# nvidia-cosmos/cosmos-curate

Hardware: AMD Instinct MI355X
Metric: clips/sec + embedded frames/sec, 1080p30 H.264, 1/2/4/8 MI355X (higher is better)
Workload: dtype bf16; 1 GPU; split_pipeline 1xMI355X: HIP NV12->RGB/resize + CLIP-ViT-B/32 MFMA bf16 (decode seam excluded: no librocdecode in image); model=vit_b32, frames_per_clip=21, src=1080p30 NV12 in HBM, resolution=224, parallelism=dp1

## Files before the change

### cosmos_curate_amd/csrc/cc_attn.hip

```cpp

#include <hip/hip_runtime.h>

#include <vector>

#include "cc_common.hpp"
#include "cc_timing.hpp"

namespace {

typedef __attribute__((ext_vector_type(8))) __bf16 bf16x8;
typedef __attribute__((ext_vector_type(4))) float f32x4;

constexpr int SMAX = 64;
constexpr int HD = 64;
constexpr int LD = 72;

__global__ __launch_bounds__(256, 2) void k_attn_small(
    const __bf16* __restrict__ qkv, __bf16* __restrict__ out, long n_frames,
    int seq, int heads, int hidden, float scale) {
  const long fh = blockIdx.x;
  const long frame = fh / heads;
  const int head = fh % heads;
  if (frame >= n_frames) return;

// ... 370 lines not shown
        m_run[reg] = mx;
#pragma unroll
        for (int nn = 0; nn < 4; nn++) acc[nn][reg] = sv[nn];
      }
    }
    {
      const int colr = lane & 15;
      const int rb = 16 * wid + rbase_l;
#pragma unroll
      for (int nn = 0; nn < 4; nn++)
#pragma unroll
        for (int reg = 0; reg < 4; reg++)
          P[(rb + reg) * LDF + nn * 16 + colr] = (__bf16)acc[nn][reg];
    }
    __syncthreads();

    f32x4 pv[4] = {};
    {
      const int prow = 16 * wid + (lane & 15);
      const int j0 = 8 * (lane >> 4);
#pragma unroll
      for (int kk = 0; kk < FKV; kk += 32) {
        bf16x8 pf = *(const bf16x8*)(P + prow * LDF + kk + j0);
#pragma unroll
        for (int n = 0; n < 4; n++) {
          bf16x8 vf =
              *(const bf16x8*)(Vt + (n * 16 + (lane & 15)) * LDF + kk + j0);
          pv[n] = __builtin_amdgcn_mfma_f32_16x16x32_bf16(pf, vf, pv[n], 0, 0, 0);
        }
      }
    }
#pragma unroll
    for (int n = 0; n < 4; n++)
#pragma unroll
      for (int reg = 0; reg < 4; reg++)
        oacc[n][reg] = oacc[n][reg] * alpha[reg] + pv[n][reg];
  }

  {
    const int dcol = lane & 15;
    const int rb = 16 * wid + rbase_l;
#pragma unroll
    for (int nn = 0; nn < 4; nn++)
#pragma unroll
      for (int reg = 0; reg < 4; reg++) {
        const int row = q0 + rb + reg;
        if (row < seq)
          out[(frame * seq + row) * (long)hidden + head * HD + nn * 16 + dcol] =
              (__bf16)(oacc[nn][reg] / l_run[reg]);
      }
  }
}

}

extern "C" int cc_attn_small(const void* qkv, void* out, int64_t n_frames,
                             int seq, int heads, int hidden, float scale,
                             uint64_t stream) {
  if (!qkv || !out || n_frames <= 0 || seq <= 0)
    return cc::set_error(CC_ERR_INVALID, "bad attn args");
  if (seq > SMAX || hidden != heads * HD)
    return cc::set_error(CC_ERR_UNSUPPORTED,
                         "cc_attn_small needs seq <= 64 and hd == 64");
  dim3 block(256), grid((unsigned)(n_frames * heads));
  hipEvent_t ev0, ev1;
  bool timed = cc::timed_begin(stream, &ev0, &ev1);
  hipLaunchKernelGGL(k_attn_small, grid, block, 0, (hipStream_t)stream,
                     (const __bf16*)qkv, (__bf16*)out, (long)n_frames, seq,
                     heads, hidden, scale);
  hipError_t e = hipGetLastError();
  if (timed) cc::timed_end("attn_small", stream, ev0, ev1);
  if (e != hipSuccess)
    return cc::set_error(CC_ERR_HIP, "attn launch: %s", hipGetErrorString(e));
  return CC_OK;
}

extern "C" int cc_attn_mid(const void* qkv, void* out, int64_t n_frames,
                           int seq, int heads, int hidden, float scale,
                           uint64_t stream) {
  if (!qkv || !out || n_frames <= 0 || seq <= 0)
    return cc::set_error(CC_ERR_INVALID, "bad attn args");
  if (seq <= SMAX || seq > SMID || hidden != heads * HD)
    return cc::set_error(CC_ERR_UNSUPPORTED,
                         "cc_attn_mid needs 64 < seq <= 288 and hd == 64");
  dim3 block(256), grid((unsigned)(n_frames * heads));
  hipEvent_t ev0, ev1;
  bool timed = cc::timed_begin(stream, &ev0, &ev1);
  hipLaunchKernelGGL(k_attn_mid, grid, block, 0, (hipStream_t)stream,
                     (const __bf16*)qkv, (__bf16*)out, (long)n_frames, seq,
                     heads, hidden, scale);
  hipError_t e = hipGetLastError();
  if (timed) cc::timed_end("attn_mid", stream, ev0, ev1);
  if (e != hipSuccess)
    return cc::set_error(CC_ERR_HIP, "attn_mid launch: %s", hipGetErrorString(e));
  return CC_OK;
}

extern "C" int cc_attn_flash(const void* qkv, void* out, int64_t n_frames,
                             int seq, int heads, int hidden, float scale,
                             uint64_t stream) {
  if (!qkv || !out || n_frames <= 0 || seq <= 0)
    return cc::set_error(CC_ERR_INVALID, "bad attn args");
  if (seq <= SMID || hidden != heads * HD)
    return cc::set_error(CC_ERR_UNSUPPORTED,
                         "cc_attn_flash is for seq > 288 with hd == 64 "
                         "(use attn_small/attn_mid below that)");
// ... 14 lines not shown
```

### cosmos_curate_amd/csrc/cc_gemm.hip

```cpp

#include <hip/hip_runtime.h>

#include <cstdlib>
#include <vector>

#include "cc_common.hpp"
#include "cc_timing.hpp"

#define CC_CHECK_HIP(expr)                                                   \
  do {                                                                       \
    hipError_t _e = (expr);                                                  \
    if (_e != hipSuccess)                                                    \
      return cc::set_error(CC_ERR_HIP, "%s failed: %s", #expr,               \
                           hipGetErrorString(_e));                           \
  } while (0)

namespace {

typedef __attribute__((ext_vector_type(8))) __bf16 bf16x8;
typedef __attribute__((ext_vector_type(4))) float f32x4;
typedef __attribute__((ext_vector_type(16))) float f32x16;

constexpr int BM = 128, BN = 128, BK = 64;
constexpr int WM = 64, WN = 64;
// ... 1 lines not shown
constexpr int MFR = WM / FRAG;
constexpr int NFR = WN / FRAG;

__device__ __forceinline__ unsigned short f32_to_bf16_rne(float v) {
  union {
    float f;
    unsigned int u;
  } cv{v};
  unsigned int lsb = (cv.u >> 16) & 1;
  return (unsigned short)((cv.u + 0x7fffu + lsb) >> 16);
}

template <int ACT>
__device__ __forceinline__ float cc_act(float v) {
  if constexpr (ACT == 1)
    return v * __builtin_amdgcn_rcpf(1.0f + __expf(-1.702f * v));
  if constexpr (ACT == 2) {
    float z = 0.7978845608028654f * (v + 0.044715f * v * v * v);
    float t = 1.0f - 2.0f * __builtin_amdgcn_rcpf(__expf(2.0f * z) + 1.0f);
    return 0.5f * v * (1.0f + t);
  }
  return v;
}

__device__ __forceinline__ void stage_slice(const __bf16* __restrict__ src,
                                            long ld, long row0, long row_limit,
                                            long k0, __bf16* lds_base,
                                            int lane) {
  const int lrow8 = lane >> 3;
  const int slot = lane & 7;
  const int gk16 = slot ^ lrow8;
#pragma unroll
  for (int j = 0; j < 4; j++) {
    long grow = row0 + j * 8 + lrow8;
    grow = grow < 0 ? 0 : (grow >= row_limit ? row_limit - 1 : grow);
    const __bf16* gptr = src + grow * ld + k0 + (long)gk16 * 8;
    __builtin_amdgcn_global_load_lds(
        (const __attribute__((address_space(1))) unsigned int*)gptr,
        (__attribute__((address_space(3))) unsigned int*)(lds_base + j * 8 * BK),
        16, 0, 0);
  }
}

__device__ __forceinline__ bf16x8 frag_read(const __bf16* tile, int row,
                                            int k16) {
  int slot = k16 ^ (row & 7);
  return *(const bf16x8*)(tile + (long)row * BK + slot * 8);
}

template <int ACT, bool HAS_BIAS, bool HAS_RES>
__global__ __launch_bounds__(256, 2) void k_gemm_bf16(
    const __bf16* __restrict__ A, const __bf16* __restrict__ B,
    void* __restrict__ C, const float* __restrict__ bias,
    const __bf16* __restrict__ residual, long M, long N, long K,
    int c_is_bf16, int nbx, int nwg, int do_remap) {
  __shared__ __bf16 lds[2 * (BM + BN) * BK];
#define AS(b) (lds + (b) * (BM * BK))
#define BS(b) (lds + 2 * (BM * BK) + (b) * (BN * BK))

  const int tid = threadIdx.x;
  const int lane = tid & 63;
  const int wid = tid >> 6;
  const int waveM = wid >> 1, waveN = wid & 1;

  int orig = blockIdx.x;
  if (do_remap) {
    int q = nwg >> 3, r = nwg & 7;
    int xcd = orig & 7, lid = orig >> 3;
    orig = (xcd < r ? xcd * (q + 1) : r * (q + 1) + (xcd - r) * q) + lid;
  }
  const long bm = (long)(orig / nbx) * BM;
  const long bn = (long)(orig % nbx) * BN;

  const long arow0 = bm + 32 * wid;
  const long brow0 = bn + 32 * wid;

  f32x4 acc[MFR][NFR] = {};

  const long KT = K / BK;
  stage_slice(A, K, arow0, M, 0, AS(0) + 32 * wid * BK, lane);
  stage_slice(B, K, brow0, N, 0, BS(0) + 32 * wid * BK, lane);

  const int arow_frag = waveM * WM + (lane & 15);
  const int brow_frag = waveN * WN + (lane & 15);
  int buf = 0;
  for (long kt = 0; kt < KT; ++kt) {
    asm volatile("s_waitcnt vmcnt(0)" ::: "memory");
    __syncthreads();
    const __bf16* At = AS(buf);
    const __bf16* Bt = BS(buf);
    bf16x8 afrag[2][MFR], bfrag[2][NFR];
#pragma unroll
    for (int g = 0; g < 2; g++) {
      const int k16 = (g << 2) + (lane >> 4);
#pragma unroll
      for (int m = 0; m < MFR; m++)
        afrag[g][m] = frag_read(At, arow_frag + m * FRAG, k16);
#pragma unroll
      for (int n = 0; n < NFR; n++)
        bfrag[g][n] = frag_read(Bt, brow_frag + n * FRAG, k16);
    }
    if (kt + 1 < KT) {
      const long k0 = (kt + 1) * BK;
      stage_slice(A, K, arow0, M, k0, AS(buf ^ 1) + 32 * wid * BK, lane);
      stage_slice(B, K, brow0, N, k0, BS(buf ^ 1) + 32 * wid * BK, lane);
    }
#pragma unroll
    for (int g = 0; g < 2; g++)
#pragma unroll
      for (int m = 0; m < MFR; m++)
#pragma unroll
        for (int n = 0; n < NFR; n++)
          acc[m][n] = __builtin_amdgcn_mfma_f32_16x16x32_bf16(
              afrag[g][m], bfrag[g][n], acc[m][n], 0, 0, 0);
    buf ^= 1;
  }

  const long crow_base = bm + waveM * WM + 4 * (lane >> 4);
  const long ccol_base = bn + waveN * WN + (lane & 15);
  const bool interior = (bm + BM <= M) && (bn + BN <= N);
  if (interior) {
#pragma unroll
    for (int m = 0; m < MFR; m++) {
#pragma unroll
      for (int n = 0; n < NFR; n++) {
        const long col = ccol_base + n * FRAG;
        float bval = 0.0f;
        if constexpr (HAS_BIAS) bval = bias[col];
        float rv[4];
        if constexpr (HAS_RES) {
#pragma unroll
          for (int r = 0; r < 4; r++)
            rv[r] = (float)residual[(crow_base + m * FRAG + r) * N + col];
        }
#pragma unroll
        for (int r = 0; r < 4; r++) {
          const long row = crow_base + m * FRAG + r;
          float v = acc[m][n][r] + bval;
          if (ACT == 1) v = v * __builtin_amdgcn_rcpf(1.0f + __expf(-1.702f * v));
          if (ACT == 2) {
            float z = 0.7978845608028654f * (v + 0.044715f * v * v * v);
            float t = 1.0f - 2.0f * __builtin_amdgcn_rcpf(__expf(2.0f * z) + 1.0f);
            v = 0.5f * v * (1.0f + t);
          }
          if constexpr (HAS_RES) v += rv[r];
          if (c_is_bf16)
            ((unsigned short*)C)[row * N + col] = f32_to_bf16_rne(v);
          else
            ((float*)C)[row * N + col] = v;
        }
      }
    }
    return;
  }
#pragma unroll
  for (int m = 0; m < MFR; m++) {
#pragma unroll
    for (int n = 0; n < NFR; n++) {
      const long col = ccol_base + n * FRAG;
      if (col >= N) continue;
      float bval = 0.0f;
      if constexpr (HAS_BIAS) bval = bias[col];
#pragma unroll
      for (int r = 0; r < 4; r++) {
        const long row = crow_base + m * FRAG + r;
        if (row >= M) continue;
        float v = acc[m][n][r] + bval;
        if (ACT == 1) v = v * __builtin_amdgcn_rcpf(1.0f + __expf(-1.702f * v));
        if (ACT == 2) {
          float z = 0.7978845608028654f * (v + 0.044715f * v * v * v);
          float t = 1.0f - 2.0f * __builtin_amdgcn_rcpf(__expf(2.0f * z) + 1.0f);
          v = 0.5f * v * (1.0f + t);
        }
        if constexpr (HAS_RES) v += (float)residual[row * N + col];
        if (c_is_bf16)
          ((unsigned short*)C)[row * N + col] = f32_to_bf16_rne(v);
        else
          ((float*)C)[row * N + col] = v;
      }
    }
  }
}

template <int ACT, bool HAS_BIAS, bool HAS_RES>
__global__ __launch_bounds__(256, 2) void k_gemm_bf16_w32(
    const __bf16* __restrict__ A, const __bf16* __restrict__ B,
    void* __restrict__ C, const float* __restrict__ bias,
    const __bf16* __restrict__ residual, long M, long N, long K,
    int c_is_bf16, int nbx, int nwg, int do_remap) {
  __shared__ __bf16 lds[2 * (BM + BN) * BK];
#define AS32(b) (lds + (b) * (BM * BK))
#define BS32(b) (lds + 2 * (BM * BK) + (b) * (BN * BK))
  const int tid = threadIdx.x;
  const int lane = tid & 63;
  const int wid = tid >> 6;
  const int waveM = wid >> 1, waveN = wid & 1;

  int orig = blockIdx.x;
  if (do_remap) {
    int q = nwg >> 3, r = nwg & 7;
    int xcd = orig & 7, lid = orig >> 3;
    orig = (xcd < r ? xcd * (q + 1) : r * (q + 1) + (xcd - r) * q) + lid;
  }
  const long bm = (long)(orig / nbx) * BM;
  const long bn = (long)(orig % nbx) * BN;
  const long arow0 = bm + 32 * wid;
  const long brow0 = bn + 32 * wid;

  f32x16 acc[2][2] = {};
  const long KT = K / BK;
  stage_slice(A, K, arow0, M, 0, AS32(0) + 32 * wid * BK, lane);
  stage_slice(B, K, brow0, N, 0, BS32(0) + 32 * wid * BK, lane);
  const int arow = waveM * WM + (lane & 31);
  const int brow = waveN * WN + (lane & 31);
  int buf = 0;
  for (long kt = 0; kt < KT; ++kt) {
    asm volatile("s_waitcnt vmcnt(0)" ::: "memory");
    __syncthreads();
    if (kt + 1 < KT) {
      const long k0 = (kt + 1) * BK;
      stage_slice(A, K, arow0, M, k0, AS32(buf ^ 1) + 32 * wid * BK, lane);
      stage_slice(B, K, brow0, N, k0, BS32(buf ^ 1) + 32 * wid * BK, lane);
    }
    const __bf16* At = AS32(buf);
    const __bf16* Bt = BS32(buf);
#pragma unroll
    for (int kk = 0; kk < BK; kk += 16) {
// ... 315 lines not shown
          bf16x8 v8 = *(const bf16x8*)(slice + elem);
          if constexpr (HAS_RES) {
            const bf16x8 r8 =
                *(const bf16x8*)(residual + grow * N + gcol);
#pragma unroll
            for (int e = 0; e < 8; e++)
              v8[e] = (__bf16)((float)v8[e] + (float)r8[e]);
          }
          *(bf16x8*)((__bf16*)C + grow * N + gcol) = v8;
        }
      }
    } else {
      const bool interior = (ebm + BM2 <= M) && (ebn + BN2 <= N);
      float bhoist2[NFR2] = {};
      if constexpr (HAS_BIAS) {
#pragma unroll
        for (int n = 0; n < NFR2; n++) {
          const long col = ccol_base + n * FRAG;
          bhoist2[n] = (interior || col < N) ? bias[col] : 0.0f;
        }
      }
#pragma unroll
      for (int m = 0; m < MFR2; m++) {
#pragma unroll
        for (int n = 0; n < NFR2; n++) {
          const long col = ccol_base + n * FRAG;
          if (!interior && col >= N) continue;
          const float bval = bhoist2[n];
#pragma unroll
          for (int r = 0; r < 4; r++) {
            const long row = crow_base + m * FRAG + r;
            if (!interior && row >= M) continue;
            float v = cc_act<ACT>(acc[m][n][r] + bval);
            if constexpr (HAS_RES) v += (float)residual[row * N + col];
            if (c_is_bf16)
              ((unsigned short*)C)[row * N + col] = f32_to_bf16_rne(v);
            else
              ((float*)C)[row * N + col] = v;
          }
        }
      }
    }
  }
#undef A2T
#undef B2T
#undef STAGE_A2
#undef STAGE_B2
#undef PHASE_MFMA2
#undef READ_A2
#undef READ_B2
#undef KTILE2
}

}

extern "C" int cc_gemm_bf16_ex(const void* A, const void* B, void* C,
                               int64_t M, int64_t N, int64_t K,
                               const float* bias, int c_dtype, int act,
                               const void* residual, uint64_t stream) {
  if (!A || !B || !C || M <= 0 || N <= 0 || K <= 0)
    return cc::set_error(CC_ERR_INVALID, "bad gemm args");
  if (K % BK != 0)
    return cc::set_error(CC_ERR_UNSUPPORTED,
                         "cc_gemm_bf16 requires K %% 64 == 0 (got %lld)",
                         (long long)K);
  int nbx = (int)((N + BN - 1) / BN);
  int nby = (int)((M + BM - 1) / BM);
  int nwg = nbx * nby;
  dim3 block(256);
  dim3 grid(nwg);
  hipEvent_t ev0 = nullptr, ev1 = nullptr;
  bool timed = cc::timed_begin(stream, &ev0, &ev1);
  static const int wide_env = [] {
    const char* e = getenv("CC_GEMM_WIDE");
    return e ? atoi(e) : -1;
  }();
  const bool wide = wide_env >= 0 ? wide_env != 0 : false;
  static const int tile_env = [] {
    const char* e = getenv("CC_GEMM_TILE");
    return e ? atoi(e) : -1;
  }();
  const bool t256_ok = (K % 128 == 0) && (K >= 256) && M > BM2 / 2;
  const int nbx2 = (int)((N + BN2 - 1) / BN2);
  const int nby2 = (int)((M + BM2 - 1) / BM2);
  const int nwg2 = nbx2 * nby2;
  const bool t256 =
      !wide && t256_ok &&
      (tile_env >= 0 ? tile_env != 0
                     : (K >= 1536 || N >= 1536 || nwg2 >= 256));
  const bool hb = bias != nullptr;
  const bool hr = residual != nullptr;
  int remap = ((M * N) > (48LL << 20)) ? 1 : 0;
  if (t256) {
    nbx = nbx2;
    nby = nby2;
    nwg = nwg2;
    static const int persist_env = [] {
      const char* e = getenv("CC_GEMM_PERSIST");
      return e ? atoi(e) : 1;
    }();
    grid = dim3(persist_env && nwg > 256 ? 256 : nwg);
    block = dim3(512);
    remap = nbx <= 16 ? 1 : 0;
  }
  static const int epi_env = [] {
    const char* e = getenv("CC_GEMM_EPI");
    return e ? atoi(e) : -1;
  }();
  const int epi_auto = (bias != nullptr || residual != nullptr || act != 0) ? 1 : 0;
  const bool epi_staged = (epi_env >= 0 ? epi_env : epi_auto) != 0;
#define CC_LAUNCH_GEMM(KER, A_, HB, HR)                                       \
  hipLaunchKernelGGL((KER<A_, HB, HR>), grid, block, 0, (hipStream_t)stream,  \
                     (const __bf16*)A, (const __bf16*)B, C, bias,             \
                     (const __bf16*)residual, (long)M, (long)N, (long)K,      \
                     c_dtype == 1 ? 1 : 0, nbx, nwg, remap)
#define CC_LAUNCH_T256(A_, HB, HR)                                            \
  do {                                                                        \
    if (epi_staged)                                                           \
      hipLaunchKernelGGL((k_gemm_bf16_t256<A_, HB, HR, true>), grid, block,   \
                         0, (hipStream_t)stream, (const __bf16*)A,            \
                         (const __bf16*)B, C, bias, (const __bf16*)residual,  \
                         (long)M, (long)N, (long)K, c_dtype == 1 ? 1 : 0,     \
                         nbx, nwg, remap);                                    \
    else                                                                      \
      hipLaunchKernelGGL((k_gemm_bf16_t256<A_, HB, HR, false>), grid, block,  \
                         0, (hipStream_t)stream, (const __bf16*)A,            \
                         (const __bf16*)B, C, bias, (const __bf16*)residual,  \
                         (long)M, (long)N, (long)K, c_dtype == 1 ? 1 : 0,     \
                         nbx, nwg, remap);                                    \
  } while (0)
#define CC_DISPATCH_ACT(KER, A_)                                              \
  do {                                                                        \
    if (hb && hr) CC_LAUNCH_GEMM(KER, A_, true, true);                        \
    else if (hb) CC_LAUNCH_GEMM(KER, A_, true, false);                        \
    else if (hr) CC_LAUNCH_GEMM(KER, A_, false, true);                        \
    else CC_LAUNCH_GEMM(KER, A_, false, false);                               \
  } while (0)
#define CC_DISPATCH(KER)                                                      \
  do {                                                                        \
    if (act == 1) CC_DISPATCH_ACT(KER, 1);                                    \
    else if (act == 2) CC_DISPATCH_ACT(KER, 2);       \
    else CC_DISPATCH_ACT(KER, 0);                                             \
  } while (0)
  if (wide)
    CC_DISPATCH(k_gemm_bf16_w32);
  else if (t256) {
#define CC_DISPATCH_ACT_T256(A_)                                              \
  do {                                                                        \
    if (hb && hr) CC_LAUNCH_T256(A_, true, true);                             \
    else if (hb) CC_LAUNCH_T256(A_, true, false);                             \
    else if (hr) CC_LAUNCH_T256(A_, false, true);                             \
    else CC_LAUNCH_T256(A_, false, false);                                    \
  } while (0)
    if (act == 1) CC_DISPATCH_ACT_T256(1);
    else if (act == 2) CC_DISPATCH_ACT_T256(2);
    else CC_DISPATCH_ACT_T256(0);
#undef CC_DISPATCH_ACT_T256
  } else
    CC_DISPATCH(k_gemm_bf16);
#undef CC_DISPATCH
#undef CC_DISPATCH_ACT
#undef CC_LAUNCH_GEMM
  hipError_t e = hipGetLastError();
  if (timed) cc::timed_end("gemm_bf16", stream, ev0, ev1);
  if (e != hipSuccess)
    return cc::set_error(CC_ERR_HIP, "gemm launch: %s", hipGetErrorString(e));
  return CC_OK;
}

extern "C" int cc_gemm_bf16(const void* A, const void* B, void* C, int64_t M,
                            int64_t N, int64_t K, const float* bias,
                            int c_dtype, uint64_t stream) {
  return cc_gemm_bf16_ex(A, B, C, M, N, K, bias, c_dtype, 0, nullptr, stream);
}
```

### cosmos_curate_amd/hotpath.py

```python

from __future__ import annotations

import ctypes
import pathlib

import numpy as np
import numpy.typing as npt

_LIB_PATH = pathlib.Path(__file__).resolve().parent / "lib" / "libcchot.so"
_lib: ctypes.CDLL | None = None


class HotpathUnavailableError(RuntimeError):
    """libcchot.so missing or unusable — the product GPU path must not run."""


def _declare(lib: ctypes.CDLL) -> None:
    c = ctypes
    lib.cc_last_error.restype = c.c_char_p
    lib.cc_hip_available.restype = c.c_int
    lib.cc_rocdecode_available.restype = c.c_int

    lib.cc_demux_open.argtypes = [c.c_char_p, c.c_size_t, c.POINTER(c.c_void_p)]
    lib.cc_demux_probe.argtypes = [c.c_void_p, c.c_void_p]
    lib.cc_demux_timestamps.argtypes = [
        c.c_void_p, c.c_void_p, c.c_size_t, c.POINTER(c.c_size_t)]
    lib.cc_demux_packet.argtypes = [
        c.c_void_p, c.c_size_t, c.POINTER(c.c_void_p), c.POINTER(c.c_size_t),
        c.POINTER(c.c_int64), c.POINTER(c.c_int32)]
    lib.cc_demux_close.argtypes = [c.c_void_p]
    lib.cc_demux_remux_clip.argtypes = [
        c.c_void_p, c.c_double, c.c_double, c.POINTER(c.c_void_p),
        c.POINTER(c.c_size_t)]
    lib.cc_buffer_free.argtypes = [c.c_void_p]

    lib.cc_decode_session_create.argtypes = [
        c.c_int, c.c_int32, c.POINTER(c.c_void_p)]
    lib.cc_decode_submit.argtypes = [
        c.c_void_p, c.c_char_p, c.c_size_t, c.c_int64]
    lib.cc_decode_map_frames.argtypes = [
        c.c_void_p, c.c_void_p, c.c_size_t, c.POINTER(c.c_size_t)]
    lib.cc_decode_recycle.argtypes = [c.c_void_p]
    lib.cc_decode_destroy.argtypes = [c.c_void_p]

    lib.cc_malloc.argtypes = [c.POINTER(c.c_void_p), c.c_size_t]
    lib.cc_free.argtypes = [c.c_void_p]
    lib.cc_memcpy_h2d.argtypes = [c.c_void_p, c.c_void_p, c.c_size_t, c.c_uint64]
    lib.cc_memcpy_d2h.argtypes = [c.c_void_p, c.c_void_p, c.c_size_t, c.c_uint64]
    lib.cc_stream_sync.argtypes = [c.c_uint64]

    lib.cc_nv12_to_rgb.argtypes = [
        c.c_void_p, c.c_void_p, c.c_int, c.c_int, c.c_int, c.c_size_t,
        c.c_void_p, c.c_uint64]
    lib.cc_nv12_to_rgb_resize.argtypes = [
        c.c_void_p, c.c_void_p, c.c_int, c.c_int, c.c_int, c.c_size_t,
        c.c_void_p, c.c_int, c.c_int, c.c_uint64]
    lib.cc_resize_bilinear_u8.argtypes = [
        c.c_void_p, c.c_int, c.c_int, c.c_int, c.c_void_p, c.c_int, c.c_int,
        c.c_uint64]
    lib.cc_resize_bicubic_u8.argtypes = lib.cc_resize_bilinear_u8.argtypes
    lib.cc_clip_preprocess.argtypes = [
        c.c_void_p, c.c_int, c.c_int, c.c_int, c.POINTER(c.c_float),
        c.POINTER(c.c_float), c.c_void_p, c.c_int, c.c_uint64]
    lib.cc_clip_preprocess_patches.argtypes = [
        c.c_void_p, c.c_int, c.c_int, c.c_int, c.c_int, c.c_int,
        c.POINTER(c.c_float), c.POINTER(c.c_float), c.c_void_p, c.c_uint64]
    lib.cc_gather_frames_u8.argtypes = [
        c.c_void_p, c.c_int, c.c_size_t, c.c_void_p, c.c_void_p, c.c_int,
        c.c_int, c.c_void_p, c.c_uint64]
    lib.cc_gemm_bf16.argtypes = [
        c.c_void_p, c.c_void_p, c.c_void_p, c.c_int64, c.c_int64, c.c_int64,
        c.c_void_p, c.c_int, c.c_uint64]
    lib.cc_gemm_bf16_ex.argtypes = [
        c.c_void_p, c.c_void_p, c.c_void_p, c.c_int64, c.c_int64, c.c_int64,
        c.c_void_p, c.c_int, c.c_int, c.c_void_p, c.c_uint64]

    lib.cc_attn_small.argtypes = [
        c.c_void_p, c.c_void_p, c.c_int64, c.c_int, c.c_int, c.c_int,
        c.c_float, c.c_uint64]
    lib.cc_attn_mid.argtypes = lib.cc_attn_small.argtypes
    lib.cc_attn_flash.argtypes = lib.cc_attn_small.argtypes
    lib.cc_layernorm_bf16.argtypes = [
        c.c_void_p, c.c_void_p, c.c_void_p, c.c_void_p, c.c_int64, c.c_int64,
        c.c_float, c.c_uint64]
    lib.cc_embed_assemble_ln.argtypes = [
        c.c_void_p, c.c_void_p, c.c_void_p, c.c_void_p, c.c_void_p,
        c.c_void_p, c.c_int64, c.c_int64, c.c_int64, c.c_float, c.c_uint64]
    lib.cc_pairwise_max_earlier.argtypes = [
        c.c_void_p, c.c_int64, c.c_int64, c.c_void_p, c.c_void_p, c.c_uint64]

    lib.cc_timing_enable.argtypes = [c.c_int]
    lib.cc_timing_report.argtypes = [
        c.c_char_p, c.POINTER(c.c_double), c.POINTER(c.c_int64)]


def load() -> ctypes.CDLL:
    global _lib
    if _lib is None:
        if not _LIB_PATH.exists():
            raise HotpathUnavailableError(
                f"{_LIB_PATH} not built — run python -m cosmos_curate_amd.build"
            )
        _lib = ctypes.CDLL(str(_LIB_PATH))
        _declare(_lib)
    return _lib


def available() -> bool:
    try:
        load()
    except HotpathUnavailableError:
        return False
    return True


def require_gpu() -> ctypes.CDLL:
    lib = load()
    rc = lib.cc_hip_available()
    if rc != 0:
        raise HotpathUnavailableError(
            f"HIP device unavailable: {lib.cc_last_error().decode()}"
        )
    return lib


def check(rc: int) -> None:
    if rc != 0:
        lib = load()
        raise RuntimeError(f"cc error {rc}: {lib.cc_last_error().decode()}")
# ... 147 lines not shown
```

### cosmos_curate_amd/models/clip_vit.py

```python

from __future__ import annotations

import ctypes
import math

import torch

from cosmos_curate_amd import hotpath
from cosmos_curate_amd.models import clip_weights as cw


def _cc_linear(
    x: torch.Tensor,
    w_bf16: torch.Tensor,
    bias_f32: torch.Tensor | None,
    act: int = 0,
    residual: torch.Tensor | None = None,
) -> torch.Tensor:
    lib = hotpath.require_gpu()
    assert x.dtype == torch.bfloat16 and w_bf16.dtype == torch.bfloat16
    x = x.contiguous()
    M, K = x.shape
    N = w_bf16.shape[0]
    out = torch.empty((M, N), dtype=torch.bfloat16, device=x.device)
    stream = torch.cuda.current_stream(x.device).cuda_stream
    if residual is not None:
        residual = residual.contiguous()
        assert residual.shape == out.shape and residual.dtype == torch.bfloat16
    hotpath.check(
        lib.cc_gemm_bf16_ex(
            x.data_ptr(), w_bf16.data_ptr(), out.data_ptr(), M, N, K,
            bias_f32.data_ptr() if bias_f32 is not None else None,
            1, act, residual.data_ptr() if residual is not None else None,
            stream,
        )
    )
    return out


class ClipVisionTowerAMD(torch.nn.Module):

    def __init__(
        self,
        state_dict: dict[str, torch.Tensor] | None = None,
        cfg: cw.VitConfig = cw.VIT_B32,
    ) -> None:
        super().__init__()
        self.cfg = cfg
        if state_dict is None:
            state_dict = (
                cw.make_clip_vit_b32_weights() if cfg is cw.VIT_B32
                else cw.make_clip_vit_weights(cfg)
            )
        sd = state_dict
        p = "vision_model."
        reg = self.register_buffer
        to_bf = lambda t: t.to(torch.bfloat16).contiguous()

        k0 = 3 * cfg.patch * cfg.patch
        self.patch_k = (k0 + 63) // 64 * 64
        reg("cls_emb", sd[p + "embeddings.class_embedding"].clone())
        w_patch = sd[p + "embeddings.patch_embedding.weight"].reshape(cfg.hidden, k0)
        if self.patch_k != k0:
            w_patch = torch.nn.functional.pad(w_patch, (0, self.patch_k - k0))
        reg("w_patch", to_bf(w_patch))
        reg("pos_emb", sd[p + "embeddings.position_embedding.weight"].clone())
        reg("pre_ln_w", sd[p + "pre_layrnorm.weight"].clone())
        reg("pre_ln_b", sd[p + "pre_layrnorm.bias"].clone())
        self.layers = cfg.layers
        for i in range(self.layers):
            q = f"{p}encoder.layers.{i}."
            wq, wk, wv = (sd[q + f"self_attn.{x}.weight"] for x in ("q_proj", "k_proj", "v_proj"))
            bq, bk, bv = (sd[q + f"self_attn.{x}.bias"] for x in ("q_proj", "k_proj", "v_proj"))
            reg(f"w_qkv_{i}", to_bf(torch.cat([wq, wk, wv], dim=0)))
            reg(f"b_qkv_{i}", torch.cat([bq, bk, bv]).float().contiguous())
            reg(f"w_out_{i}", to_bf(sd[q + "self_attn.out_proj.weight"]))
            reg(f"b_out_{i}", sd[q + "self_attn.out_proj.bias"].float().contiguous())
            reg(f"ln1_w_{i}", sd[q + "layer_norm1.weight"].clone())
            reg(f"ln1_b_{i}", sd[q + "layer_norm1.bias"].clone())
            reg(f"ln2_w_{i}", sd[q + "layer_norm2.weight"].clone())
            reg(f"ln2_b_{i}", sd[q + "layer_norm2.bias"].clone())
            reg(f"w_fc1_{i}", to_bf(sd[q + "mlp.fc1.weight"]))
            reg(f"b_fc1_{i}", sd[q + "mlp.fc1.bias"].float().contiguous())
            reg(f"w_fc2_{i}", to_bf(sd[q + "mlp.fc2.weight"]))
            reg(f"b_fc2_{i}", sd[q + "mlp.fc2.bias"].float().contiguous())
        reg("post_ln_w", sd[p + "post_layernorm.weight"].clone())
        reg("post_ln_b", sd[p + "post_layernorm.bias"].clone())
        reg("w_proj", to_bf(sd["visual_projection.weight"]))
        self.heads = cfg.heads
        self.scale = 1.0 / math.sqrt(cfg.hidden // cfg.heads)

    def _linear(
        self,
# ... 17 lines not shown
                lib.cc_layernorm_bf16(
                    xc.data_ptr(), w.data_ptr(), b.data_ptr(), out.data_ptr(),
                    m, h, 1e-5, stream,
                )
            )
            return out
        return torch.nn.functional.layer_norm(
            x.float(), (x.shape[-1],), w, b, eps=1e-5
        ).to(x.dtype)

    @torch.no_grad()
    def forward(
        self,
        pixel_values: torch.Tensor | None = None,
        *,
        patches: torch.Tensor | None = None,
        n: int | None = None,
    ) -> torch.Tensor:
        cfg = self.cfg
        g = cfg.image // cfg.patch
        k0 = 3 * cfg.patch * cfg.patch
        if patches is None:
            x = pixel_values.to(torch.bfloat16)
            n = x.shape[0]
            patches = (
                x.reshape(n, 3, g, cfg.patch, g, cfg.patch)
                .permute(0, 2, 4, 1, 3, 5)
                .reshape(n * g * g, k0)
            )
            if self.patch_k != k0:
                patches = torch.nn.functional.pad(patches, (0, self.patch_k - k0))
        else:
            assert n is not None and patches.shape == (n * g * g, self.patch_k)
        tok_flat = self._linear(patches, self.w_patch, None)
        seq = g * g + 1
        if tok_flat.is_cuda:
            lib = hotpath.require_gpu()
            h = torch.empty((n * seq, cfg.hidden), dtype=torch.bfloat16,
                            device=tok_flat.device)
            stream = torch.cuda.current_stream(tok_flat.device).cuda_stream
            hotpath.check(lib.cc_embed_assemble_ln(
                tok_flat.data_ptr(), self.cls_emb.data_ptr(),
                self.pos_emb.data_ptr(), self.pre_ln_w.data_ptr(),
                self.pre_ln_b.data_ptr(), h.data_ptr(), n, seq, cfg.hidden,
                ctypes.c_float(1e-5), stream))
            h = h.reshape(n, seq, cfg.hidden)
        else:
            tok = tok_flat.reshape(n, g * g, cfg.hidden)
            cls = self.cls_emb.to(tok.dtype).expand(n, 1, cfg.hidden)
            h = torch.cat([cls, tok], dim=1)
            h = (h.float() + self.pos_emb.unsqueeze(0)).to(torch.bfloat16)
            h = self._ln(h, self.pre_ln_w, self.pre_ln_b)
        hd = cfg.hidden // self.heads
        for i in range(self.layers):
            res = h
            y = self._ln(h, getattr(self, f"ln1_w_{i}"), getattr(self, f"ln1_b_{i}"))
            qkv_flat = self._linear(
                y.reshape(n * seq, cfg.hidden),
                getattr(self, f"w_qkv_{i}"),
                getattr(self, f"b_qkv_{i}"),
            )
            if qkv_flat.is_cuda and hd == 64:
                lib = hotpath.require_gpu()
                attn = torch.empty(
                    (n * seq, cfg.hidden), dtype=torch.bfloat16,
                    device=qkv_flat.device,
                )
                stream = torch.cuda.current_stream(qkv_flat.device).cuda_stream
                attn_fn = (lib.cc_attn_small if seq <= 64 else
                           lib.cc_attn_mid if seq <= 288 else
                           lib.cc_attn_flash)
                hotpath.check(
                    attn_fn(
                        qkv_flat.data_ptr(), attn.data_ptr(), n, seq,
                        self.heads, cfg.hidden, ctypes.c_float(self.scale),
                        stream,
                    )
                )
            else:
                qkv = qkv_flat.reshape(n, seq, 3, self.heads, hd)
                q = qkv[:, :, 0].permute(0, 2, 1, 3)
                k = qkv[:, :, 1].permute(0, 2, 1, 3)
                v = qkv[:, :, 2].permute(0, 2, 1, 3)
                attn = torch.nn.functional.scaled_dot_product_attention(
                    q, k, v, scale=self.scale
                )
                attn = attn.permute(0, 2, 1, 3).reshape(n * seq, cfg.hidden)
            h = self._linear(
                attn, getattr(self, f"w_out_{i}"), getattr(self, f"b_out_{i}"),
                residual=res.reshape(n * seq, cfg.hidden),
            ).reshape(n, seq, cfg.hidden)

            res = h
            y = self._ln(h, getattr(self, f"ln2_w_{i}"), getattr(self, f"ln2_b_{i}"))
            y = self._linear(
                y.reshape(n * seq, cfg.hidden),
                getattr(self, f"w_fc1_{i}"),
                getattr(self, f"b_fc1_{i}"),
                act=1,
            )
            h = self._linear(
                y, getattr(self, f"w_fc2_{i}"), getattr(self, f"b_fc2_{i}"),
                residual=res.reshape(n * seq, cfg.hidden),
            ).reshape(n, seq, cfg.hidden)

        pooled = self._ln(h[:, 0], self.post_ln_w, self.post_ln_b)
        emb = self._linear(pooled.to(torch.bfloat16), self.w_proj, None).float()
        return emb / torch.linalg.vector_norm(emb, dim=-1, keepdim=True)
```

### include/cc_hotpath.h

```cpp

#ifndef CC_HOTPATH_H
#define CC_HOTPATH_H

#include <stddef.h>
#include <stdint.h>

#ifdef __cplusplus
extern "C" {
#endif

enum {
  CC_OK = 0,
  CC_ERR_INVALID = -1,
  CC_ERR_PARSE = -2,
  CC_ERR_NOMEM = -3,
  CC_ERR_HIP = -4,
  CC_ERR_NO_ROCDECODE = -5,
  CC_ERR_UNSUPPORTED = -6,
};

const char* cc_last_error(void);

int cc_hip_available(void);
int cc_rocdecode_available(void);
// ... 15 lines not shown
int  cc_demux_timestamps(const cc_demux_t* d, float* out, size_t cap, size_t* n);
int  cc_demux_packet(cc_demux_t* d, size_t index, const uint8_t** pkt,
                     size_t* size, int64_t* pts, int32_t* keyframe);
void cc_demux_close(cc_demux_t* d);
int  cc_demux_remux_clip(cc_demux_t* d, double start_s, double end_s,
                         uint8_t** out, size_t* out_size);
void cc_buffer_free(void* p);

int cc_malloc(void** dptr, size_t bytes);
int cc_free(void* dptr);
int cc_memcpy_h2d(void* dst, const void* src, size_t bytes, uint64_t stream);
int cc_memcpy_d2h(void* dst, const void* src, size_t bytes, uint64_t stream);
int cc_stream_sync(uint64_t stream);

typedef struct cc_decode cc_decode_t;
int  cc_decode_session_create(int device, int32_t codec, cc_decode_t** out);
int  cc_decode_submit(cc_decode_t* s, const uint8_t* pkt, size_t size, int64_t pts);
typedef struct cc_nv12_frame {
  void* y; void* uv; size_t pitch; int64_t pts; uint32_t width, height;
} cc_nv12_frame;
int  cc_decode_map_frames(cc_decode_t* s, cc_nv12_frame* out, size_t cap, size_t* n);
int  cc_decode_recycle(cc_decode_t* s);
void cc_decode_destroy(cc_decode_t* s);


int cc_nv12_to_rgb_resize(const void* y, const void* uv, int n,
                          int src_h, int src_w, size_t pitch,
                          void* out_rgb, int out_h, int out_w,
                          uint64_t stream);
int cc_nv12_to_rgb(const void* y, const void* uv, int n,
                   int h, int w, size_t pitch, void* out_rgb, uint64_t stream);
int cc_resize_bilinear_u8(const void* in, int n, int src_h, int src_w,
                          void* out, int dst_h, int dst_w, uint64_t stream);
int cc_resize_bicubic_u8(const void* in, int n, int src_h, int src_w,
                         void* out, int dst_h, int dst_w, uint64_t stream);
int cc_clip_preprocess(const void* in, int n, int h, int w,
                       const float mean[3], const float stdev[3],
                       void* out, int out_dtype, uint64_t stream);
int cc_clip_preprocess_patches(const void* in, int n, int h, int w, int patch,
                               int kpad, const float mean[3],
                               const float stdev[3], void* out,
                               uint64_t stream);
int cc_gather_frames_u8(const void* frames, int n_in, size_t frame_bytes,
                        const int32_t* idx, const int32_t* counts, int n_idx,
                        int total_out, void* out, uint64_t stream);

int cc_gemm_bf16(const void* A, const void* B, void* C,
                 int64_t M, int64_t N, int64_t K,
                 const float* bias, int c_dtype, uint64_t stream);
int cc_gemm_bf16_ex(const void* A, const void* B, void* C,
                    int64_t M, int64_t N, int64_t K,
                    const float* bias, int c_dtype, int act,
                    const void* residual, uint64_t stream);

int cc_attn_small(const void* qkv, void* out, int64_t n_frames, int seq,
                  int heads, int hidden, float scale, uint64_t stream);

int cc_attn_mid(const void* qkv, void* out, int64_t n_frames, int seq,
                int heads, int hidden, float scale, uint64_t stream);

int cc_attn_flash(const void* qkv, void* out, int64_t n_frames, int seq,
                  int heads, int hidden, float scale, uint64_t stream);

int cc_layernorm_bf16(const void* x, const void* w, const void* b, void* y,
                      int64_t M, int64_t H, float eps, uint64_t stream);

int cc_embed_assemble_ln(const void* tok, const void* cls, const void* pos,
                         const void* w, const void* b, void* y,
                         int64_t n_frames, int64_t tokens, int64_t H,
                         float eps, uint64_t stream);

int cc_pairwise_max_earlier(const void* e_f32, int64_t m, int64_t d,
                            void* maxv_f32, void* argi_i32, uint64_t stream);

int cc_timing_enable(int enable);
int cc_timing_reset(void);
int cc_timing_report(const char* kernel, double* total_ms, int64_t* count);

#ifdef __cplusplus
}
#endif
#endif
```

Baseline: 4516 clips/s.

## Prune last ViT layer to CLS token with strided GEMM and CLS attention kernel

In the final transformer layer, only the CLS row feeds the pooled embedding. So the change computes K/V for all tokens but Q, attention output projection, MLP and residual only for the CLS row. A new wave-per-head CLS attention kernel reads strided K/V from the fused kv buffer. The GEMM gains lda/ldr strides so strided views can be consumed without copies, and a tile-selection tweak avoids underfilled 256 tiles. This drops roughly the last layer's MLP and projection work for non-CLS tokens, at the cost of extra small launches and new code paths.

```diff
diff --git a/cosmos_curate_amd/csrc/cc_attn.hip b/cosmos_curate_amd/csrc/cc_attn.hip
--- a/cosmos_curate_amd/csrc/cc_attn.hip
+++ b/cosmos_curate_amd/csrc/cc_attn.hip
@@ -446,6 +446,124 @@
   }
 }
 
+__global__ __launch_bounds__(256) void k_attn_cls(
+    const __bf16* __restrict__ q, const __bf16* __restrict__ k,
+    const __bf16* __restrict__ v, long ldkv, __bf16* __restrict__ out,
+    long n_frames, int seq, int heads, int hidden, float scale) {
+  const int lane = threadIdx.x & 63;
+  const long fh = (long)blockIdx.x * 4 + (threadIdx.x >> 6);
+  if (fh >= n_frames * heads) return;
+  const long frame = fh / heads;
+  const int head = (int)(fh % heads);
+  const int jg = lane >> 3;
+  const int dg = lane & 7;
+
+  float qf[8];
+  {
+    const bf16x8 q8 =
+        *(const bf16x8*)(q + frame * (long)hidden + head * HD + dg * 8);
+#pragma unroll
+    for (int e = 0; e < 8; e++) qf[e] = (float)q8[e] * scale;
+  }
+  const long kv_base = frame * (long)seq * ldkv + (long)head * HD + dg * 8;
+
+  float m_run = -1e30f, l_run = 0.0f;
+  float oacc[8] = {};
+  for (int k0 = 0; k0 < seq; k0 += 64) {
+    bf16x8 kr[8], vr[8];
+#pragma unroll
+    for (int jj = 0; jj < 8; jj++) {
+      int j = k0 + jj * 8 + jg;
+      j = j < seq ? j : seq - 1;
+      kr[jj] = *(const bf16x8*)(k + kv_base + (long)j * ldkv);
+      vr[jj] = *(const bf16x8*)(v + kv_base + (long)j * ldkv);
+    }
+    float s[8];
+    float mx = m_run;
+#pragma unroll
+    for (int jj = 0; jj < 8; jj++) {
+      float d = 0.0f;
+#pragma unroll
+      for (int e = 0; e < 8; e++) d += qf[e] * (float)kr[jj][e];
+      d += __shfl_xor(d, 1);
+      d += __shfl_xor(d, 2);
+      d += __shfl_xor(d, 4);
+      if (k0 + jj * 8 + jg >= seq) d = -1e30f;
+      s[jj] = d;
+      mx = fmaxf(mx, d);
+    }
+    mx = fmaxf(mx, __shfl_xor(mx, 8));
+    mx = fmaxf(mx, __shfl_xor(mx, 16));
+    mx = fmaxf(mx, __shfl_xor(mx, 32));
+    const float alpha = __expf(m_run - mx);
+    float sum = 0.0f;
+    float pv[8] = {};
+#pragma unroll
+    for (int jj = 0; jj < 8; jj++) {
+      const bool live = k0 + jj * 8 + jg < seq;
+      const float e = live ? __expf(s[jj] - mx) : 0.0f;
+      sum += e;
+      const float p = (float)(__bf16)e;
+#pragma unroll
+      for (int d = 0; d < 8; d++)
+        pv[d] += live ? p * (float)vr[jj][d] : 0.0f;
+    }
+    sum += __shfl_xor(sum, 8);
+    sum += __shfl_xor(sum, 16);
+    sum += __shfl_xor(sum, 32);
+    l_run = l_run * alpha + sum;
+    m_run = mx;
+#pragma unroll
+    for (int d = 0; d < 8; d++) oacc[d] = oacc[d] * alpha + pv[d];
+  }
+#pragma unroll
+  for (int d = 0; d < 8; d++) {
+    float o = oacc[d];
+    o += __shfl_xor(o, 8);
+    o += __shfl_xor(o, 16);
+    o += __shfl_xor(o, 32);
+    oacc[d] = o;
+  }
+  if (jg == 0) {
+    const float inv = 1.0f / l_run;
+    bf16x8 o8;
+#pragma unroll
+    for (int d = 0; d < 8; d++) o8[d] = (__bf16)(oacc[d] * inv);
+    *(bf16x8*)(out + frame * (long)hidden + head * HD + dg * 8) = o8;
+  }
+}
+
+}
+
+extern "C" int cc_attn_cls(const void* q, const void* k, const void* v,
+                           int64_t ldkv, void* out, int64_t n_frames, int seq,
+                           int heads, int hidden, float scale,
+                           uint64_t stream) {
+  if (!q || !k || !v || !out || n_frames <= 0 || seq <= 0 || heads <= 0)
+    return cc::set_error(CC_ERR_INVALID, "bad attn_cls args");
+  if (hidden != heads * HD)
+    return cc::set_error(CC_ERR_UNSUPPORTED, "cc_attn_cls needs hd == 64");
+  if (ldkv < hidden || ldkv % 8 != 0 || ((uintptr_t)q & 15) ||
+      ((uintptr_t)k & 15) || ((uintptr_t)v & 15) || ((uintptr_t)out & 15))
+    return cc::set_error(CC_ERR_INVALID,
+                         "cc_attn_cls needs ldkv >= hidden, ldkv %% 8 == 0 "
+                         "and 16-byte aligned q/k/v/out");
+  const int64_t nwave = n_frames * heads;
+  if ((nwave + 3) / 4 > 0x7fffffffLL)
+    return cc::set_error(CC_ERR_INVALID, "attn_cls grid too large");
+  dim3 block(256), grid((unsigned)((nwave + 3) / 4));
+  hipEvent_t ev0, ev1;
+  bool timed = cc::timed_begin(stream, &ev0, &ev1);
+  hipLaunchKernelGGL(k_attn_cls, grid, block, 0, (hipStream_t)stream,
+                     (const __bf16*)q, (const __bf16*)k, (const __bf16*)v,
+                     (long)ldkv, (__bf16*)out, (long)n_frames, seq, heads,
+                     hidden, scale);
+  hipError_t e = hipGetLastError();
+  if (timed) cc::timed_end("attn_cls", stream, ev0, ev1);
+  if (e != hipSuccess)
+    return cc::set_error(CC_ERR_HIP, "attn_cls launch: %s",
+                         hipGetErrorString(e));
+  return CC_OK;
 }
 
 extern "C" int cc_attn_small(const void* qkv, void* out, int64_t n_frames,
diff --git a/cosmos_curate_amd/csrc/cc_gemm.hip b/cosmos_curate_amd/csrc/cc_gemm.hip
--- a/cosmos_curate_amd/csrc/cc_gemm.hip
+++ b/cosmos_curate_amd/csrc/cc_gemm.hip
@@ -77,8 +77,8 @@
 __global__ __launch_bounds__(256, 2) void k_gemm_bf16(
     const __bf16* __restrict__ A, const __bf16* __restrict__ B,
     void* __restrict__ C, const float* __restrict__ bias,
-    const __bf16* __restrict__ residual, long M, long N, long K,
-    int c_is_bf16, int nbx, int nwg, int do_remap) {
+    const __bf16* __restrict__ residual, long M, long N, long K, long lda,
+    long ldr, int c_is_bf16, int nbx, int nwg, int do_remap) {
   __shared__ __bf16 lds[2 * (BM + BN) * BK];
 #define AS(b) (lds + (b) * (BM * BK))
 #define BS(b) (lds + 2 * (BM * BK) + (b) * (BN * BK))
@@ -103,7 +103,7 @@
   f32x4 acc[MFR][NFR] = {};
 
   const long KT = K / BK;
-  stage_slice(A, K, arow0, M, 0, AS(0) + 32 * wid * BK, lane);
+  stage_slice(A, lda, arow0, M, 0, AS(0) + 32 * wid * BK, lane);
   stage_slice(B, K, brow0, N, 0, BS(0) + 32 * wid * BK, lane);
 
   const int arow_frag = waveM * WM + (lane & 15);
@@ -127,7 +127,7 @@
     }
     if (kt + 1 < KT) {
       const long k0 = (kt + 1) * BK;
-      stage_slice(A, K, arow0, M, k0, AS(buf ^ 1) + 32 * wid * BK, lane);
+      stage_slice(A, lda, arow0, M, k0, AS(buf ^ 1) + 32 * wid * BK, lane);
       stage_slice(B, K, brow0, N, k0, BS(buf ^ 1) + 32 * wid * BK, lane);
     }
 #pragma unroll
@@ -156,7 +156,7 @@
         if constexpr (HAS_RES) {
 #pragma unroll
           for (int r = 0; r < 4; r++)
-            rv[r] = (float)residual[(crow_base + m * FRAG + r) * N + col];
+            rv[r] = (float)residual[(crow_base + m * FRAG + r) * ldr + col];
         }
 #pragma unroll
         for (int r = 0; r < 4; r++) {
@@ -197,7 +197,7 @@
           float t = 1.0f - 2.0f * __builtin_amdgcn_rcpf(__expf(2.0f * z) + 1.0f);
           v = 0.5f * v * (1.0f + t);
         }
-        if constexpr (HAS_RES) v += (float)residual[row * N + col];
+        if constexpr (HAS_RES) v += (float)residual[row * ldr + col];
         if (c_is_bf16)
           ((unsigned short*)C)[row * N + col] = f32_to_bf16_rne(v);
         else
@@ -619,18 +619,28 @@
 #undef KTILE2
 }
 
-}
-
-extern "C" int cc_gemm_bf16_ex(const void* A, const void* B, void* C,
-                               int64_t M, int64_t N, int64_t K,
-                               const float* bias, int c_dtype, int act,
-                               const void* residual, uint64_t stream) {
+int gemm_launch(const void* A, int64_t lda, const void* B, void* C, int64_t M,
+                int64_t N, int64_t K, const float* bias, int c_dtype, int act,
+                const void* residual, int64_t ldr, uint64_t stream) {
   if (!A || !B || !C || M <= 0 || N <= 0 || K <= 0)
     return cc::set_error(CC_ERR_INVALID, "bad gemm args");
   if (K % BK != 0)
     return cc::set_error(CC_ERR_UNSUPPORTED,
                          "cc_gemm_bf16 requires K %% 64 == 0 (got %lld)",
                          (long long)K);
+  if (!residual) ldr = N;
+  if (lda < K || ldr < N)
+    return cc::set_error(CC_ERR_INVALID,
+                         "gemm row stride below row length (lda %lld < K "
+                         "%lld or ldr %lld < N %lld)",
+                         (long long)lda, (long long)K, (long long)ldr,
+                         (long long)N);
+  if (lda % 8 != 0)
+    return cc::set_error(CC_ERR_INVALID,
+                         "gemm lda %lld breaks the 16-byte alignment of the "
+                         "direct-to-LDS loads (needs lda %% 8 == 0)",
+                         (long long)lda);
+  const bool strided = lda != K || ldr != N;
   int nbx = (int)((N + BN - 1) / BN);
   int nby = (int)((M + BM - 1) / BM);
   int nwg = nbx * nby;
@@ -642,7 +652,7 @@
     const char* e = getenv("CC_GEMM_WIDE");
     return e ? atoi(e) : -1;
   }();
-  const bool wide = wide_env >= 0 ? wide_env != 0 : false;
+  const bool wide = !strided && (wide_env >= 0 ? wide_env != 0 : false);
   static const int tile_env = [] {
     const char* e = getenv("CC_GEMM_TILE");
     return e ? atoi(e) : -1;
@@ -651,10 +661,12 @@
   const int nbx2 = (int)((N + BN2 - 1) / BN2);
   const int nby2 = (int)((M + BM2 - 1) / BM2);
   const int nwg2 = nbx2 * nby2;
+  const bool underfill = N < 1536 && nwg2 < 128 && nwg >= 128;
   const bool t256 =
-      !wide && t256_ok &&
-      (tile_env >= 0 ? tile_env != 0
-                     : (K >= 1536 || N >= 1536 || nwg2 >= 256));
+      !wide && !strided && t256_ok &&
+      (tile_env >= 0
+           ? tile_env != 0
+           : ((K >= 1536 && !underfill) || N >= 1536 || nwg2 >= 256));
   const bool hb = bias != nullptr;
   const bool hr = residual != nullptr;
   int remap = ((M * N) > (48LL << 20)) ? 1 : 0;
@@ -681,6 +693,12 @@
                      (const __bf16*)A, (const __bf16*)B, C, bias,             \
                      (const __bf16*)residual, (long)M, (long)N, (long)K,      \
                      c_dtype == 1 ? 1 : 0, nbx, nwg, remap)
+#define CC_LAUNCH_GEMM_LD(KER, A_, HB, HR)                                    \
+  hipLaunchKernelGGL((KER<A_, HB, HR>), grid, block, 0, (hipStream_t)stream,  \
+                     (const __bf16*)A, (const __bf16*)B, C, bias,             \
+                     (const __bf16*)residual, (long)M, (long)N, (long)K,      \
+                     (long)lda, (long)ldr, c_dtype == 1 ? 1 : 0, nbx, nwg,    \
+                     remap)
 #define CC_LAUNCH_T256(A_, HB, HR)                                            \
   do {                                                                        \
     if (epi_staged)                                                           \
@@ -696,21 +714,21 @@
                          (long)M, (long)N, (long)K, c_dtype == 1 ? 1 : 0,     \
                          nbx, nwg, remap);                                    \
   } while (0)
-#define CC_DISPATCH_ACT(KER, A_)                                              \
+#define CC_DISPATCH_ACT(L, KER, A_)                                           \
   do {                                                                        \
-    if (hb && hr) CC_LAUNCH_GEMM(KER, A_, true, true);                        \
-    else if (hb) CC_LAUNCH_GEMM(KER, A_, true, false);                        \
-    else if (hr) CC_LAUNCH_GEMM(KER, A_, false, true);                        \
-    else CC_LAUNCH_GEMM(KER, A_, false, false);                               \
+    if (hb && hr) L(KER, A_, true, true);                                     \
+    else if (hb) L(KER, A_, true, false);                                     \
+    else if (hr) L(KER, A_, false, true);                                     \
+    else L(KER, A_, false, false);                                            \
   } while (0)
-#define CC_DISPATCH(KER)                                                      \
+#define CC_DISPATCH(L, KER)                                                   \
   do {                                                                        \
-    if (act == 1) CC_DISPATCH_ACT(KER, 1);                                    \
-    else if (act == 2) CC_DISPATCH_ACT(KER, 2);       \
-    else CC_DISPATCH_ACT(KER, 0);                                             \
+    if (act == 1) CC_DISPATCH_ACT(L, KER, 1);                                 \
+    else if (act == 2) CC_DISPATCH_ACT(L, KER, 2);    \
+    else CC_DISPATCH_ACT(L, KER, 0);                                          \
   } while (0)
   if (wide)
-    CC_DISPATCH(k_gemm_bf16_w32);
+    CC_DISPATCH(CC_LAUNCH_GEMM, k_gemm_bf16_w32);
   else if (t256) {
 #define CC_DISPATCH_ACT_T256(A_)                                              \
   do {                                                                        \
@@ -724,10 +742,11 @@
     else CC_DISPATCH_ACT_T256(0);
 #undef CC_DISPATCH_ACT_T256
   } else
-    CC_DISPATCH(k_gemm_bf16);
+    CC_DISPATCH(CC_LAUNCH_GEMM_LD, k_gemm_bf16);
 #undef CC_DISPATCH
 #undef CC_DISPATCH_ACT
 #undef CC_LAUNCH_GEMM
+#undef CC_LAUNCH_GEMM_LD
   hipError_t e = hipGetLastError();
   if (timed) cc::timed_end("gemm_bf16", stream, ev0, ev1);
   if (e != hipSuccess)
@@ -735,6 +754,25 @@
   return CC_OK;
 }
 
+}
+
+extern "C" int cc_gemm_bf16_ex(const void* A, const void* B, void* C,
+                               int64_t M, int64_t N, int64_t K,
+                               const float* bias, int c_dtype, int act,
+                               const void* residual, uint64_t stream) {
+  return gemm_launch(A, K, B, C, M, N, K, bias, c_dtype, act, residual, N,
+                     stream);
+}
+
+extern "C" int cc_gemm_bf16_strided(const void* A, int64_t lda, const void* B,
+                                    void* C, int64_t M, int64_t N, int64_t K,
+                                    const float* bias, int c_dtype, int act,
+                                    const void* residual, int64_t ldr,
+                                    uint64_t stream) {
+  return gemm_launch(A, lda, B, C, M, N, K, bias, c_dtype, act, residual, ldr,
+                     stream);
+}
+
 extern "C" int cc_gemm_bf16(const void* A, const void* B, void* C, int64_t M,
                             int64_t N, int64_t K, const float* bias,
                             int c_dtype, uint64_t stream) {
diff --git a/cosmos_curate_amd/hotpath.py b/cosmos_curate_amd/hotpath.py
--- a/cosmos_curate_amd/hotpath.py
+++ b/cosmos_curate_amd/hotpath.py
@@ -74,7 +74,14 @@
     lib.cc_gemm_bf16_ex.argtypes = [
         c.c_void_p, c.c_void_p, c.c_void_p, c.c_int64, c.c_int64, c.c_int64,
         c.c_void_p, c.c_int, c.c_int, c.c_void_p, c.c_uint64]
-
+    lib.cc_gemm_bf16_strided.argtypes = [
+        c.c_void_p, c.c_int64, c.c_void_p, c.c_void_p, c.c_int64, c.c_int64,
+        c.c_int64, c.c_void_p, c.c_int, c.c_int, c.c_void_p, c.c_int64,
+        c.c_uint64]
+
+    lib.cc_attn_cls.argtypes = [
+        c.c_void_p, c.c_void_p, c.c_void_p, c.c_int64, c.c_void_p, c.c_int64,
+        c.c_int, c.c_int, c.c_int, c.c_float, c.c_uint64]
     lib.cc_attn_small.argtypes = [
         c.c_void_p, c.c_void_p, c.c_int64, c.c_int, c.c_int, c.c_int,
         c.c_float, c.c_uint64]
diff --git a/cosmos_curate_amd/models/clip_vit.py b/cosmos_curate_amd/models/clip_vit.py
--- a/cosmos_curate_amd/models/clip_vit.py
+++ b/cosmos_curate_amd/models/clip_vit.py
@@ -19,26 +19,53 @@
 ) -> torch.Tensor:
     lib = hotpath.require_gpu()
     assert x.dtype == torch.bfloat16 and w_bf16.dtype == torch.bfloat16
-    x = x.contiguous()
+    assert w_bf16.is_contiguous()
     M, K = x.shape
     N = w_bf16.shape[0]
+    lda = _row_stride(x)
+    if lda is None or lda % 8 != 0:
+        x = x.contiguous()
+        lda = K
     out = torch.empty((M, N), dtype=torch.bfloat16, device=x.device)
     stream = torch.cuda.current_stream(x.device).cuda_stream
+    ldr = N
     if residual is not None:
-        residual = residual.contiguous()
         assert residual.shape == out.shape and residual.dtype == torch.bfloat16
-    hotpath.check(
-        lib.cc_gemm_bf16_ex(
-            x.data_ptr(), w_bf16.data_ptr(), out.data_ptr(), M, N, K,
-            bias_f32.data_ptr() if bias_f32 is not None else None,
-            1, act, residual.data_ptr() if residual is not None else None,
-            stream,
-        )
-    )
+        ldr = _row_stride(residual)
+        if ldr is None:
+            residual = residual.contiguous()
+            ldr = N
+    bias_p = bias_f32.data_ptr() if bias_f32 is not None else None
+    res_p = residual.data_ptr() if residual is not None else None
+    if lda == K and ldr == N:
+        hotpath.check(
+            lib.cc_gemm_bf16_ex(
+                x.data_ptr(), w_bf16.data_ptr(), out.data_ptr(), M, N, K,
+                bias_p, 1, act, res_p, stream,
+            )
+        )
+    else:
+        hotpath.check(
+            lib.cc_gemm_bf16_strided(
+                x.data_ptr(), lda, w_bf16.data_ptr(), out.data_ptr(), M, N, K,
+                bias_p, 1, act, res_p, ldr, stream,
+            )
+        )
     return out
 
 
+def _row_stride(t: torch.Tensor) -> int | None:
+    rows, cols = t.shape
+    if t.stride(1) != 1 and cols != 1:
+        return None
+    if rows == 1:
+        return cols
+    return t.stride(0) if t.stride(0) >= cols else None
+
+
 class ClipVisionTowerAMD(torch.nn.Module):
+
+    prune_last_layer = True
 
     def __init__(
         self,
@@ -162,7 +189,14 @@
             h = (h.float() + self.pos_emb.unsqueeze(0)).to(torch.bfloat16)
             h = self._ln(h, self.pre_ln_w, self.pre_ln_b)
         hd = cfg.hidden // self.heads
+        cls_only = (
+            self.prune_last_layer and cfg.has_cls
+            and (hd == 64 or not h.is_cuda)
+        )
         for i in range(self.layers):
+            if cls_only and i == self.layers - 1:
+                h = self._last_layer_cls(h, i, n, seq)
+                break
             res = h
             y = self._ln(h, getattr(self, f"ln1_w_{i}"), getattr(self, f"ln1_b_{i}"))
             qkv_flat = self._linear(
@@ -214,6 +248,51 @@
                 residual=res.reshape(n * seq, cfg.hidden),
             ).reshape(n, seq, cfg.hidden)
 
-        pooled = self._ln(h[:, 0], self.post_ln_w, self.post_ln_b)
+        cls_rows = h if cls_only else h[:, 0]
+        pooled = self._ln(cls_rows, self.post_ln_w, self.post_ln_b)
         emb = self._linear(pooled.to(torch.bfloat16), self.w_proj, None).float()
         return emb / torch.linalg.vector_norm(emb, dim=-1, keepdim=True)
+
+    def _last_layer_cls(
+        self, h: torch.Tensor, i: int, n: int, seq: int
+    ) -> torch.Tensor:
+        H = self.cfg.hidden
+        hd = H // self.heads
+        w_qkv = getattr(self, f"w_qkv_{i}")
+        b_qkv = getattr(self, f"b_qkv_{i}")
+        y = self._ln(h, getattr(self, f"ln1_w_{i}"), getattr(self, f"ln1_b_{i}"))
+        kv = self._linear(y.reshape(n * seq, H), w_qkv[H:], b_qkv[H:])
+        q = self._linear(y[:, 0], w_qkv[:H], b_qkv[:H])
+        if kv.is_cuda:
+            lib = hotpath.require_gpu()
+            attn = torch.empty((n, H), dtype=torch.bfloat16, device=kv.device)
+            stream = torch.cuda.current_stream(kv.device).cuda_stream
+            hotpath.check(
+                lib.cc_attn_cls(
+                    q.data_ptr(), kv.data_ptr(),
+                    kv.data_ptr() + H * kv.element_size(), 2 * H,
+                    attn.data_ptr(), n, seq, self.heads, H,
+                    ctypes.c_float(self.scale), stream,
+                )
+            )
+        else:
+            kvh = kv.reshape(n, seq, 2, self.heads, hd)
+            attn = torch.nn.functional.scaled_dot_product_attention(
+                q.reshape(n, 1, self.heads, hd).permute(0, 2, 1, 3),
+                kvh[:, :, 0].permute(0, 2, 1, 3),
+                kvh[:, :, 1].permute(0, 2, 1, 3),
+                scale=self.scale,
+            )
+            attn = attn.permute(0, 2, 1, 3).reshape(n, H)
+        h1 = self._linear(
+            attn, getattr(self, f"w_out_{i}"), getattr(self, f"b_out_{i}"),
+            residual=h[:, 0],
+        )
+        y = self._ln(h1, getattr(self, f"ln2_w_{i}"), getattr(self, f"ln2_b_{i}"))
+        y = self._linear(
+            y, getattr(self, f"w_fc1_{i}"), getattr(self, f"b_fc1_{i}"), act=1
+        )
+        return self._linear(
+            y, getattr(self, f"w_fc2_{i}"), getattr(self, f"b_fc2_{i}"),
+            residual=h1,
+        )
diff --git a/include/cc_hotpath.h b/include/cc_hotpath.h
--- a/include/cc_hotpath.h
+++ b/include/cc_hotpath.h
@@ -91,6 +91,10 @@
                     int64_t M, int64_t N, int64_t K,
                     const float* bias, int c_dtype, int act,
                     const void* residual, uint64_t stream);
+int cc_gemm_bf16_strided(const void* A, int64_t lda, const void* B, void* C,
+                         int64_t M, int64_t N, int64_t K, const float* bias,
+                         int c_dtype, int act, const void* residual,
+                         int64_t ldr, uint64_t stream);
 
 int cc_attn_small(const void* qkv, void* out, int64_t n_frames, int seq,
                   int heads, int hidden, float scale, uint64_t stream);
@@ -100,6 +104,10 @@
 
 int cc_attn_flash(const void* qkv, void* out, int64_t n_frames, int seq,
                   int heads, int hidden, float scale, uint64_t stream);
+
+int cc_attn_cls(const void* q, const void* k, const void* v, int64_t ldkv,
+                void* out, int64_t n_frames, int seq, int heads, int hidden,
+                float scale, uint64_t stream);
 
 int cc_layernorm_bf16(const void* x, const void* w, const void* b, void* y,
                       int64_t M, int64_t H, float eps, uint64_t stream);
```

New measurement: 4803 clips/s, median of 6. 1.06x the previous value.
